# rlawhdrhs/Vision-Transformer-OpenCL

Hardware: AMD Instinct MI355X
Metric: images/sec ViT-B/16 224² fp32 @batch256; % MFMA roofline; top-1 match (higher is better)
Workload: dtype f32; 1 GPU; ViT-B/16 224x224 fp32 forward, batch 256 per GPU, synthetic weights and images (BASELINE.json configs[1]); batch_per_gpu=256, global_batch=256, parallelism=dp1, lanes_per_gpu=1, prune_last_layer=False, ln_fold=True, device=AMD Radeon Graphics, arch=gfx950:sramecc+:xnack-, compute_units=256, clock_mhz=2400

## Files before the change

vision-transformer-opencl_amd/csrc/vit_attention_hd.hip:

```cpp
#include <hip/hip_runtime.h>

#include <math.h>

#include <type_traits>

#include "vit_attention.hpp"
#include "vit_hip_kernels.h"
#include "vit_split3.hpp"

namespace {

using namespace vitattn;
typedef unsigned int u32x2 __attribute__((ext_vector_type(2)));

constexpr int HD_WAVES = 4, HD_THREADS = HD_WAVES * 64;
constexpr int HD_QROWS = HD_WAVES * 32;

template <int HD, bool BF16>
struct Geo {
    typedef typename std::conditional<BF16, bf16_t, float>::type elem;
    static constexpr int VEC = BF16 ? 8 : 4;
    static constexpr int KC = BF16 ? 64 : 32;
    static constexpr int KT = KC / 32;
    static constexpr int DT = (HD + 31) / 32;
    static constexpr int HDK = BF16 ? (HD + 15) / 16 * 16 : HD;
    static constexpr int KROW = HDK + (BF16 ? 8 : 4);
    static constexpr int VROW = KC + 4;
    static constexpr int K_ELEMS = KC * KROW, V_ELEMS = DT * 32 * VROW;
    static constexpr int MIN_WAVES = BF16 && HD <= 96 ? 4 : 3;
};

template <int HD, bool BF16, bool QS>
__global__ __launch_bounds__(HD_THREADS, (Geo<HD, BF16>::MIN_WAVES)) void attention_hd_kernel(
    const typename Geo<HD, BF16>::elem *__restrict__ qkv, typename Geo<HD, BF16>::elem *__restrict__ out, int tokens, int heads, int q_rows,
    int qblocks, float scale) {
    typedef Geo<HD, BF16> G;
    typedef typename G::elem elem;
    constexpr int VEC = G::VEC, KC = G::KC, KT = G::KT, DT = G::DT, KROW = G::KROW, VROW = G::VROW;
    __shared__ __attribute__((aligned(16))) elem Ks[G::K_ELEMS];
    __shared__ __attribute__((aligned(16))) elem Vt[G::V_ELEMS];

    const int tid = threadIdx.x, lane = tid & 63, wave = tid >> 6;
    const int r = lane & 31, h = lane >> 5;
    const int image = blockIdx.x / qblocks, qblock = blockIdx.x - image * qblocks, head = blockIdx.y;
    const size_t D = (size_t)heads * HD, ld = 3 * D;
    const elem *rows = qkv + (size_t)image * tokens * ld + (size_t)head * HD;
    const elem *krows = rows + D, *vrows = rows + 2 * D;
    const int qrow0 = qblock * HD_QROWS + wave * 32;
    const bool active = qrow0 < q_rows;

    constexpr int NQ = BF16 ? G::HDK / 16 : HD / 8;
    typename std::conditional<BF16, bf16x8, f32x4>::type qf[NQ];
    {
        int qrow = qrow0 + r;
        qrow = qrow < q_rows ? qrow : q_rows - 1;
        const elem *qp = rows + (size_t)qrow * ld;
#pragma unroll
        for (int ks = 0; ks < NQ; ++ks) {
            if constexpr (BF16) {
                const int d0 = 16 * ks + 8 * h;
                u32x4 w = {0u, 0u, 0u, 0u};
                if (d0 < HD && active) w = *reinterpret_cast<const u32x4 *>(qp + d0);
                qf[ks] = __builtin_bit_cast(bf16x8, w);
            } else {
                f32x4 w = {0.0f, 0.0f, 0.0f, 0.0f};
                if (active) w = *reinterpret_cast<const f32x4 *>(qp + 8 * ks + 4 * h);
                qf[ks] = w;
            }
        }
    }

    f32x16 o[DT];
#pragma unroll
    for (int dt = 0; dt < DT; ++dt)
#pragma unroll
        for (int v = 0; v < 16; ++v) o[dt][v] = 0.0f;
    float m_run = -INFINITY, l_run = 0.0f;

    for (int key0 = 0; key0 < tokens; key0 += KC) {
        constexpr int KP = G::HDK / VEC;
        for (int i = tid; i < KC * KP; i += HD_THREADS) {
            const int row = i / KP, c = i - row * KP, key = key0 + row;
            u32x4 w = {0u, 0u, 0u, 0u};
            if (key < tokens && c * VEC < HD) w = *reinterpret_cast<const u32x4 *>(krows + (size_t)key * ld + c * VEC);
            *reinterpret_cast<u32x4 *>(Ks + row * KROW + c * VEC) = w;
        }
        constexpr int VP = HD / VEC;
        if constexpr (BF16) {
            for (int i = tid; i < (KC / 2) * VP; i += HD_THREADS) {
                const int c = i / (KC / 2), row = 2 * (i - c * (KC / 2)), key = key0 + row;
                u32x4 a = {0u, 0u, 0u, 0u}, b = {0u, 0u, 0u, 0u};
                if (key < tokens) a = *reinterpret_cast<const u32x4 *>(vrows + (size_t)key * ld + c * VEC);
                if (key + 1 < tokens) b = *reinterpret_cast<const u32x4 *>(vrows + (size_t)(key + 1) * ld + c * VEC);
#pragma unroll
                for (int j = 0; j < 4; ++j) {
                    *reinterpret_cast<unsigned *>(Vt + (c * 8 + 2 * j) * VROW + row) = (a[j] & 0xffffu) | (b[j] << 16);
                    *reinterpret_cast<unsigned *>(Vt + (c * 8 + 2 * j + 1) * VROW + row) = (a[j] >> 16) | (b[j] & 0xffff0000u);
                }
            }
        } else {
            for (int i = tid; i < KC * VP; i += HD_THREADS) {
                const int c = i / KC, row = i - c * KC, key = key0 + row;
                u32x4 w = {0u, 0u, 0u, 0u};
                if (key < tokens) w = *reinterpret_cast<const u32x4 *>(vrows + (size_t)key * ld + c * VEC);
#pragma unroll
                for (int j = 0; j < 4; ++j) Vt[(c * 4 + j) * VROW + row] = __uint_as_float(w[j]);
            }
        }
        __syncthreads();

        if (active) {
#pragma unroll
            for (int t = 0; t < KT; ++t) {
                const int tile0 = key0 + 32 * t;
                if (tile0 >= tokens) break;
                f32x16 s;
#pragma unroll
                for (int v = 0; v < 16; ++v) s[v] = 0.0f;
                const elem *kp = Ks + (32 * t + r) * KROW;
#pragma unroll
                for (int ks = 0; ks < NQ; ++ks) {
                    if constexpr (BF16) {
                        const bf16x8 kf = *reinterpret_cast<const bf16x8 *>(kp + 16 * ks + 8 * h);
                        s = __builtin_amdgcn_mfma_f32_32x32x16_bf16(kf, qf[ks], s, 0, 0, 0);
                    } else {
                        const f32x4 kf = *reinterpret_cast<const f32x4 *>(kp + 8 * ks + 4 * h);
#pragma unroll
                        for (int i = 0; i < 4; ++i) s = __builtin_amdgcn_mfma_f32_32x32x2f32(kf[i], qf[ks][i], s, 0, 0, 0);
                    }
                }
                if (tile0 + 32 > tokens) {
#pragma unroll
                    for (int v = 0; v < 16; ++v) {
                        const int key = tile0 + (v & 3) + 8 * (v >> 2) + 4 * h;
                        s[v] = key < tokens ? s[v] : -INFINITY;
                    }
                }
                float cmax = s[0];
#pragma unroll
                for (int v = 1; v < 16; ++v) cmax = fmaxf(cmax, s[v]);
                cmax = fmaxf(cmax, __shfl_xor(cmax, 32));
                constexpr float kDefer = 8.0f;
                const float m_old = m_run;
                const float m_new = (cmax - m_old) * scale > kDefer ? cmax : m_old;
                const float mneg = -m_new * scale;
                m_run = m_new;
                float sum = 0.0f;
#pragma unroll
                for (int v = 0; v < 16; ++v) {
                    s[v] = __builtin_amdgcn_exp2f(QS ? s[v] + mneg : fmaf(s[v], scale, mneg));
                    sum += s[v];
                }
                if (__any(m_new != m_old)) {
                    const float alpha = __builtin_amdgcn_exp2f((m_old - m_new) * scale);
                    l_run *= alpha;
#pragma unroll
                    for (int dt = 0; dt < DT; ++dt)
#pragma unroll
                        for (int v = 0; v < 16; ++v) o[dt][v] *= alpha;
                }
                l_run += sum;
                if constexpr (BF16) {
#pragma unroll
                    for (int s2 = 0; s2 < 2; ++s2) {
                        bf16x8 pf, pl;
#pragma unroll
                        for (int j = 0; j < 8; ++j) {
                            pf[j] = (__bf16)s[8 * s2 + j];
                            pl[j] = (__bf16)(s[8 * s2 + j] - (float)pf[j]);
                        }
#pragma unroll
                        for (int dt = 0; dt < DT; ++dt) {
                            const bf16_t *vp = Vt + (32 * dt + r) * VROW + 32 * t + 16 * s2 + 4 * h;
                            const u32x2 lo = *reinterpret_cast<const u32x2 *>(vp), hi = *reinterpret_cast<const u32x2 *>(vp + 8);
                            const u32x4 both = {lo[0], lo[1], hi[0], hi[1]};
                            o[dt] = __builtin_amdgcn_mfma_f32_32x32x16_bf16(__builtin_bit_cast(bf16x8, both), pl, o[dt], 0, 0, 0);
                            o[dt] = __builtin_amdgcn_mfma_f32_32x32x16_bf16(__builtin_bit_cast(bf16x8, both), pf, o[dt], 0, 0, 0);
                        }
                    }
                } else {
#pragma unroll
                    for (int q = 0; q < 4; ++q)
#pragma unroll
                        for (int dt = 0; dt < DT; ++dt) {
                            const f32x4 vf = *reinterpret_cast<const f32x4 *>(Vt + (32 * dt + r) * VROW + 32 * t + 8 * q + 4 * h);
#pragma unroll
                            for (int i = 0; i < 4; ++i) o[dt] = __builtin_amdgcn_mfma_f32_32x32x2f32(vf[i], s[4 * q + i], o[dt], 0, 0, 0);
                        }
                }
            }
        }
        __syncthreads();
    }

    const int qrow = qrow0 + r;
    if (active && qrow < q_rows) {
        const float inv = 1.0f / (l_run + __shfl_xor(l_run, 32));
        elem *dst = out + ((size_t)image * tokens + qrow) * D + (size_t)head * HD;
#pragma unroll
        for (int dt = 0; dt < DT; ++dt)
#pragma unroll
            for (int q = 0; q < 4; ++q) {
                const int d0 = 32 * dt + 8 * q + 4 * h;
                if (d0 < HD) {
                    if constexpr (BF16) {
                        bf16x4 w;
#pragma unroll
                        for (int i = 0; i < 4; ++i) w[i] = (__bf16)(o[dt][4 * q + i] * inv);
                        *reinterpret_cast<u32x2 *>(dst + d0) = __builtin_bit_cast(u32x2, w);
                    } else {
                        const f32x4 w = {o[dt][4 * q] * inv, o[dt][4 * q + 1] * inv, o[dt][4 * q + 2] * inv, o[dt][4 * q + 3] * inv};
                        *reinterpret_cast<f32x4 *>(dst + d0) = w;
                    }
                }
            }
    }
}

#ifndef ATT_SPLIT_WAVES
#define ATT_SPLIT_WAVES 4
#endif
#ifndef ATT_SPLIT_MINW
#define ATT_SPLIT_MINW 3
#endif
constexpr int SP_WAVES = ATT_SPLIT_WAVES, SP_THREADS = SP_WAVES * 64, SP_QROWS = SP_WAVES * 32;

__global__ __launch_bounds__(SP_THREADS, ATT_SPLIT_MINW) void attention_split_kernel(const float *__restrict__ qkv, float *__restrict__ out,
                                                                                    int tokens, int heads, int q_rows, int qblocks) {
    using vitsplit::SPLIT_TERM_A;
    using vitsplit::SPLIT_TERM_W;
    using vitsplit::split3_piece8;
    typedef Geo<64, true> G;
    constexpr int HD = 64, KC = G::KC, KT = G::KT, DT = G::DT, KROW = G::KROW, VROW = G::VROW, NQ = HD / 16;
    __shared__ __attribute__((aligned(16))) bf16_t Ks[3 * G::K_ELEMS];
    __shared__ __attribute__((aligned(16))) bf16_t Vt[3 * G::V_ELEMS];

    const int tid = threadIdx.x, lane = tid & 63, wave = tid >> 6;
    const int r = lane & 31, h = lane >> 5;
    const int image = blockIdx.x / qblocks, qblock = blockIdx.x - image * qblocks, head = blockIdx.y;
    const size_t D = (size_t)heads * HD, ld = 3 * D;
    const float *rows = qkv + (size_t)image * tokens * ld + (size_t)head * HD;
    const float *krows = rows + D, *vrows = rows + 2 * D;
    const int qrow0 = qblock * SP_QROWS + wave * 32;
    const bool active = qrow0 < q_rows;
    const f32x4 zero4 = {0.0f, 0.0f, 0.0f, 0.0f};

    bf16x8 qf[3][NQ];
    {
        int qrow = qrow0 + r;
        qrow = qrow < q_rows ? qrow : q_rows - 1;
        const float *qp = rows + (size_t)qrow * ld + 8 * h;
#pragma unroll
        for (int ks = 0; ks < NQ; ++ks) {
            f32x4 x0 = zero4, x1 = zero4;
            if (active) {
                x0 = *reinterpret_cast<const f32x4 *>(qp + 16 * ks);
                x1 = *reinterpret_cast<const f32x4 *>(qp + 16 * ks + 4);
            }
#pragma unroll
            for (int pl = 0; pl < 3; ++pl) qf[pl][ks] = __builtin_bit_cast(bf16x8, split3_piece8(x0, x1, pl));
        }
    }

    f32x16 o[DT];
#pragma unroll
    for (int dt = 0; dt < DT; ++dt)
#pragma unroll
        for (int v = 0; v < 16; ++v) o[dt][v] = 0.0f;
    float m_run = -INFINITY, l_run = 0.0f;

    constexpr int K_ITEMS = KC * (HD / 8), V_ITEMS = (KC / 2) * (HD / 8);
    constexpr int KI = (K_ITEMS + SP_THREADS - 1) / SP_THREADS;
    constexpr int V_TID0 = SP_THREADS > V_ITEMS ? SP_THREADS - V_ITEMS : 0;
    static_assert(V_ITEMS <= SP_THREADS, "one V item per thread at most");
    const int vi = tid - V_TID0;
    f32x4 kx[KI][2], vx[4];
    auto fetch = [&](int key0) {
#pragma unroll
        for (int it = 0; it < KI; ++it) {
            const int i = tid + it * SP_THREADS, row = i / (HD / 8), c = i - row * (HD / 8), key = key0 + row;
            kx[it][0] = kx[it][1] = zero4;
            if (i < K_ITEMS && key < tokens) {
                const float *p = krows + (size_t)key * ld + 8 * c;
                kx[it][0] = *reinterpret_cast<const f32x4 *>(p);
                kx[it][1] = *reinterpret_cast<const f32x4 *>(p + 4);
            }
        }
        if (vi >= 0) {
            const int c = vi / (KC / 2), key = key0 + 2 * (vi - c * (KC / 2));
#pragma unroll
            for (int j = 0; j < 4; ++j) vx[j] = zero4;
            if (key < tokens) {
                const float *p = vrows + (size_t)key * ld + 8 * c;
                vx[0] = *reinterpret_cast<const f32x4 *>(p);
                vx[1] = *reinterpret_cast<const f32x4 *>(p + 4);
            }
            if (key + 1 < tokens) {
                const float *p = vrows + (size_t)(key + 1) * ld + 8 * c;
                vx[2] = *reinterpret_cast<const f32x4 *>(p);
                vx[3] = *reinterpret_cast<const f32x4 *>(p + 4);
            }
        }
    };
    auto store = [&](bf16_t *Kd, bf16_t *Vd) {
#pragma unroll
        for (int it = 0; it < KI; ++it) {
            const int i = tid + it * SP_THREADS, row = i / (HD / 8), c = i - row * (HD / 8);
            if (i < K_ITEMS) {
#pragma unroll
                for (int pl = 0; pl < 3; ++pl)
                    *reinterpret_cast<u32x4 *>(Kd + pl * G::K_ELEMS + row * KROW + 8 * c) = split3_piece8(kx[it][0], kx[it][1], pl);
            }
        }
        if (vi >= 0) {
            const int c = vi / (KC / 2), row = 2 * (vi - c * (KC / 2));
#pragma unroll
            for (int pl = 0; pl < 3; ++pl) {
                const u32x4 a = split3_piece8(vx[0], vx[1], pl), b = split3_piece8(vx[2], vx[3], pl);
                bf16_t *vd = Vd + pl * G::V_ELEMS + (c * 8) * VROW + row;
#pragma unroll
                for (int j = 0; j < 4; ++j) {
                    *reinterpret_cast<unsigned *>(vd + (2 * j) * VROW) = (a[j] & 0xffffu) | (b[j] << 16);
                    *reinterpret_cast<unsigned *>(vd + (2 * j + 1) * VROW) = (a[j] >> 16) | (b[j] & 0xffff0000u);
                }
            }
        }
    };

    for (int key0 = 0; key0 < tokens; key0 += KC) {
        fetch(key0);
        store(Ks, Vt);
        __syncthreads();

        if (active) {
#pragma unroll
            for (int t = 0; t < KT; ++t) {
                const int tile0 = key0 + 32 * t;
                if (tile0 >= tokens) break;
                f32x16 s;
#pragma unroll
                for (int v = 0; v < 16; ++v) s[v] = 0.0f;
                const bf16_t *kp = Ks + (32 * t + r) * KROW + 8 * h;
#pragma unroll
                for (int ks = 0; ks < NQ; ++ks) {
                    bf16x8 kf[3];
#pragma unroll
                    for (int pl = 0; pl < 3; ++pl) kf[pl] = *reinterpret_cast<const bf16x8 *>(kp + pl * G::K_ELEMS + 16 * ks);
#pragma unroll
                    for (int term = 0; term < 6; ++term)
                        s = __builtin_amdgcn_mfma_f32_32x32x16_bf16(kf[SPLIT_TERM_A[term]], qf[SPLIT_TERM_W[term]][ks], s, 0, 0, 0);
                }
                if (tile0 + 32 > tokens) {
#pragma unroll
                    for (int v = 0; v < 16; ++v) {
                        const int key = tile0 + (v & 3) + 8 * (v >> 2) + 4 * h;
                        s[v] = key < tokens ? s[v] : -INFINITY;
                    }
                }
                float cmax = s[0];
#pragma unroll
                for (int v = 1; v < 16; ++v) cmax = fmaxf(cmax, s[v]);
                cmax = fmaxf(cmax, __shfl_xor(cmax, 32));
                constexpr float kDefer = 8.0f, scale = kScale64;
                const float m_old = m_run;
                const float m_new = (cmax - m_old) * scale > kDefer ? cmax : m_old;
                const float mneg = -m_new * scale;
                m_run = m_new;
                float sum = 0.0f;
#pragma unroll
                for (int v = 0; v < 16; ++v) {
                    s[v] = __builtin_amdgcn_exp2f(fmaf(s[v], scale, mneg));
                    sum += s[v];
                }
                if (__any(m_new != m_old)) {
                    const float alpha = __builtin_amdgcn_exp2f((m_old - m_new) * scale);
                    l_run *= alpha;
#pragma unroll
                    for (int dt = 0; dt < DT; ++dt)
#pragma unroll
                        for (int v = 0; v < 16; ++v) o[dt][v] *= alpha;
                }
                l_run += sum;
#pragma unroll
                for (int s2 = 0; s2 < 2; ++s2) {
                    if (tile0 + 16 * s2 >= tokens) break;
                    f32x4 x0 = {s[8 * s2], s[8 * s2 + 1], s[8 * s2 + 2], s[8 * s2 + 3]};
                    f32x4 x1 = {s[8 * s2 + 4], s[8 * s2 + 5], s[8 * s2 + 6], s[8 * s2 + 7]};
                    bf16x8 pf[3], vf[DT][3];
#pragma unroll
                    for (int pl = 0; pl < 3; ++pl) pf[pl] = __builtin_bit_cast(bf16x8, split3_piece8(x0, x1, pl));
#pragma unroll
                    for (int dt = 0; dt < DT; ++dt)
#pragma unroll
                        for (int pl = 0; pl < 3; ++pl) {
                            const bf16_t *vp = Vt + pl * G::V_ELEMS + (32 * dt + r) * VROW + 32 * t + 16 * s2 + 4 * h;
                            const u32x2 lo = *reinterpret_cast<const u32x2 *>(vp), hi = *reinterpret_cast<const u32x2 *>(vp + 8);
                            const u32x4 both = {lo[0], lo[1], hi[0], hi[1]};
                            vf[dt][pl] = __builtin_bit_cast(bf16x8, both);
                        }
#pragma unroll
                    for (int term = 0; term < 6; ++term)
#pragma unroll
                        for (int dt = 0; dt < DT; ++dt)
                            o[dt] = __builtin_amdgcn_mfma_f32_32x32x16_bf16(vf[dt][SPLIT_TERM_A[term]], pf[SPLIT_TERM_W[term]], o[dt], 0, 0, 0);
                }
            }
        }
        __syncthreads();
    }

    const int qrow = qrow0 + r;
    if (active && qrow < q_rows) {
        const float inv = 1.0f / (l_run + __shfl_xor(l_run, 32));
        float *dst = out + ((size_t)image * tokens + qrow) * D + (size_t)head * HD + 4 * h;
#pragma unroll
        for (int dt = 0; dt < DT; ++dt)
#pragma unroll
            for (int q = 0; q < 4; ++q) {
                const f32x4 w = {o[dt][4 * q] * inv, o[dt][4 * q + 1] * inv, o[dt][4 * q + 2] * inv, o[dt][4 * q + 3] * inv};
                *reinterpret_cast<f32x4 *>(dst + 32 * dt + 8 * q) = w;
            }
    }
}

template <bool BF16, bool QS>
int launch_hd(hipStream_t s, const typename Geo<128, BF16>::elem *qkv, typename Geo<128, BF16>::elem *out, int n_images, int tokens,
              int heads, int head_dim, int q_rows) {
    const int qblocks = (q_rows + HD_QROWS - 1) / HD_QROWS;
    if (heads > 65535 || (long long)n_images * qblocks > 0x7fffffffLL) return static_cast<int>(hipErrorInvalidValue);
    const float scale = QS ? 1.0f : vithip_qscale(head_dim);
    return dispatch_int<72, 8, 8>(head_dim, [&](auto hd) {
        hipLaunchKernelGGL((attention_hd_kernel<decltype(hd)::value, BF16, QS>), dim3((unsigned)(n_images * qblocks), (unsigned)heads),
                           dim3(HD_THREADS), 0, s, qkv, out, tokens, heads, q_rows, qblocks, scale);
        return static_cast<int>(hipGetLastError());
    });
}

}

int vitattn::attention_hd_f32(hipStream_t s, const float *qkv, float *out, int n_images, int tokens, int heads, int head_dim, int q_rows) {
    return launch_hd<false, false>(s, qkv, out, n_images, tokens, heads, head_dim, q_rows);
}

int vitattn::attention_hd_bf16(hipStream_t s, const unsigned short *qkv, unsigned short *out, int n_images, int tokens, int heads,
                               int head_dim, int q_rows, bool q_scaled) {
    return q_scaled ? launch_hd<true, true>(s, qkv, out, n_images, tokens, heads, head_dim, q_rows)
                    : launch_hd<true, false>(s, qkv, out, n_images, tokens, heads, head_dim, q_rows);
}

int vitattn::attention_split_f32(hipStream_t s, const float *qkv, float *out, int n_images, int tokens, int heads, int q_rows) {
    const int qblocks = (q_rows + SP_QROWS - 1) / SP_QROWS;
    if (heads > 65535 || (long long)n_images * qblocks > 0x7fffffffLL) return static_cast<int>(hipErrorInvalidValue);
    hipLaunchKernelGGL(attention_split_kernel, dim3((unsigned)(n_images * qblocks), (unsigned)heads), dim3(SP_THREADS), 0, s, qkv, out,
                       tokens, heads, q_rows, qblocks);
    return static_cast<int>(hipGetLastError());
}

extern "C" float vithip_qscale(int head_dim) {
    if (!vitattn::hd_accepted(head_dim)) return 0.0f;
    return (float)((1.0 / sqrt((double)head_dim)) * 1.4426950408889634074);
}
```

Before: 5749 images/sec.

## Store V row-major with swizzle and read via transposing LDS loads; use buffer loads

The split-bf16 attention kernel now stores V in shared memory in its natural key-major layout with an XOR swizzle, and builds MFMA B fragments with a transposing read helper instead of writing V transposed with scattered 32-bit LDS stores. K and V global fetches are unified so every thread loads one K and one V item per pass, using buffer loads with a bounds-limited resource in place of per-item branch checks. The aim is to cut LDS store instructions and bank conflicts and to simplify address arithmetic. It relies on the v_fragment_tr helper and hardware out-of-range zeroing, and drops the compile-time macro overrides.

```diff
diff --git a/vision-transformer-opencl_amd/csrc/vit_attention_hd.hip b/vision-transformer-opencl_amd/csrc/vit_attention_hd.hip
--- a/vision-transformer-opencl_amd/csrc/vit_attention_hd.hip
+++ b/vision-transformer-opencl_amd/csrc/vit_attention_hd.hip
@@ -217,30 +217,25 @@
     }
 }
 
-#ifndef ATT_SPLIT_WAVES
-#define ATT_SPLIT_WAVES 4
-#endif
-#ifndef ATT_SPLIT_MINW
-#define ATT_SPLIT_MINW 3
-#endif
-constexpr int SP_WAVES = ATT_SPLIT_WAVES, SP_THREADS = SP_WAVES * 64, SP_QROWS = SP_WAVES * 32;
-
-__global__ __launch_bounds__(SP_THREADS, ATT_SPLIT_MINW) void attention_split_kernel(const float *__restrict__ qkv, float *__restrict__ out,
-                                                                                    int tokens, int heads, int q_rows, int qblocks) {
+constexpr int SP_WAVES = 4, SP_THREADS = SP_WAVES * 64, SP_QROWS = SP_WAVES * 32;
+constexpr int SP_MINW = 3;
+constexpr int SP_VLD = 64;
+
+__global__ __launch_bounds__(SP_THREADS, SP_MINW) void attention_split_kernel(const float *__restrict__ qkv, float *__restrict__ out, int tokens,
+                                                                             int heads, int q_rows, int qblocks) {
     using vitsplit::SPLIT_TERM_A;
     using vitsplit::SPLIT_TERM_W;
     using vitsplit::split3_piece8;
     typedef Geo<64, true> G;
-    constexpr int HD = 64, KC = G::KC, KT = G::KT, DT = G::DT, KROW = G::KROW, VROW = G::VROW, NQ = HD / 16;
+    constexpr int HD = 64, KC = G::KC, KT = G::KT, DT = G::DT, KROW = G::KROW, NQ = HD / 16, V_ELEMS = KC * SP_VLD;
     __shared__ __attribute__((aligned(16))) bf16_t Ks[3 * G::K_ELEMS];
-    __shared__ __attribute__((aligned(16))) bf16_t Vt[3 * G::V_ELEMS];
+    __shared__ __attribute__((aligned(16))) bf16_t Vs[3 * V_ELEMS];
 
     const int tid = threadIdx.x, lane = tid & 63, wave = tid >> 6;
     const int r = lane & 31, h = lane >> 5;
     const int image = blockIdx.x / qblocks, qblock = blockIdx.x - image * qblocks, head = blockIdx.y;
     const size_t D = (size_t)heads * HD, ld = 3 * D;
     const float *rows = qkv + (size_t)image * tokens * ld + (size_t)head * HD;
-    const float *krows = rows + D, *vrows = rows + 2 * D;
     const int qrow0 = qblock * SP_QROWS + wave * 32;
     const bool active = qrow0 < q_rows;
     const f32x4 zero4 = {0.0f, 0.0f, 0.0f, 0.0f};
@@ -269,67 +264,44 @@
         for (int v = 0; v < 16; ++v) o[dt][v] = 0.0f;
     float m_run = -INFINITY, l_run = 0.0f;
 
-    constexpr int K_ITEMS = KC * (HD / 8), V_ITEMS = (KC / 2) * (HD / 8);
-    constexpr int KI = (K_ITEMS + SP_THREADS - 1) / SP_THREADS;
-    constexpr int V_TID0 = SP_THREADS > V_ITEMS ? SP_THREADS - V_ITEMS : 0;
-    static_assert(V_ITEMS <= SP_THREADS, "one V item per thread at most");
-    const int vi = tid - V_TID0;
-    f32x4 kx[KI][2], vx[4];
+    constexpr int ITEMS = KC * (HD / 8), NI = ITEMS / SP_THREADS;
+    static_assert(ITEMS % SP_THREADS == 0, "every thread has an item of K and one of V in every pass");
+    f32x4 kx[NI][2], vx[NI][2];
+    unsigned xoff[NI];
+#pragma unroll
+    for (int it = 0; it < NI; ++it) {
+        const int j = tid + it * SP_THREADS;
+        xoff[it] = 4u * ((unsigned)(j >> 3) * (unsigned)ld + (unsigned)D + 8u * (j & 7));
+    }
+    const unsigned v_ofs = 4u * (unsigned)D;
     auto fetch = [&](int key0) {
-#pragma unroll
-        for (int it = 0; it < KI; ++it) {
-            const int i = tid + it * SP_THREADS, row = i / (HD / 8), c = i - row * (HD / 8), key = key0 + row;
-            kx[it][0] = kx[it][1] = zero4;
-            if (i < K_ITEMS && key < tokens) {
-                const float *p = krows + (size_t)key * ld + 8 * c;
-                kx[it][0] = *reinterpret_cast<const f32x4 *>(p);
-                kx[it][1] = *reinterpret_cast<const f32x4 *>(p + 4);
-            }
-        }
-        if (vi >= 0) {
-            const int c = vi / (KC / 2), key = key0 + 2 * (vi - c * (KC / 2));
-#pragma unroll
-            for (int j = 0; j < 4; ++j) vx[j] = zero4;
-            if (key < tokens) {
-                const float *p = vrows + (size_t)key * ld + 8 * c;
-                vx[0] = *reinterpret_cast<const f32x4 *>(p);
-                vx[1] = *reinterpret_cast<const f32x4 *>(p + 4);
-            }
-            if (key + 1 < tokens) {
-                const float *p = vrows + (size_t)(key + 1) * ld + 8 * c;
-                vx[2] = *reinterpret_cast<const f32x4 *>(p);
-                vx[3] = *reinterpret_cast<const f32x4 *>(p + 4);
-            }
+        const int valid = tokens - key0 < KC ? tokens - key0 : KC;
+        const unsigned bytes = 4u * ((unsigned)(valid - 1) * (unsigned)ld + 2u * (unsigned)D + HD);
+        const __amdgpu_buffer_rsrc_t rs = __builtin_amdgcn_make_buffer_rsrc(const_cast<float *>(rows + (size_t)key0 * ld), 0, (int)bytes, 0x00020000);
+#pragma unroll
+        for (int it = 0; it < NI; ++it) {
+            kx[it][0] = __builtin_bit_cast(f32x4, __builtin_amdgcn_raw_buffer_load_b128(rs, xoff[it], 0, 0));
+            kx[it][1] = __builtin_bit_cast(f32x4, __builtin_amdgcn_raw_buffer_load_b128(rs, xoff[it], 16, 0));
+            vx[it][0] = __builtin_bit_cast(f32x4, __builtin_amdgcn_raw_buffer_load_b128(rs, xoff[it], v_ofs, 0));
+            vx[it][1] = __builtin_bit_cast(f32x4, __builtin_amdgcn_raw_buffer_load_b128(rs, xoff[it], v_ofs + 16, 0));
         }
     };
-    auto store = [&](bf16_t *Kd, bf16_t *Vd) {
-#pragma unroll
-        for (int it = 0; it < KI; ++it) {
-            const int i = tid + it * SP_THREADS, row = i / (HD / 8), c = i - row * (HD / 8);
-            if (i < K_ITEMS) {
-#pragma unroll
-                for (int pl = 0; pl < 3; ++pl)
-                    *reinterpret_cast<u32x4 *>(Kd + pl * G::K_ELEMS + row * KROW + 8 * c) = split3_piece8(kx[it][0], kx[it][1], pl);
-            }
-        }
-        if (vi >= 0) {
-            const int c = vi / (KC / 2), row = 2 * (vi - c * (KC / 2));
+    auto store = [&]() {
+#pragma unroll
+        for (int it = 0; it < NI; ++it) {
+            const int j = tid + it * SP_THREADS, row = j >> 3, c = j & 7;
+            bf16_t *kd = Ks + row * KROW + 8 * c, *vd = Vs + row * SP_VLD + 8 * (c ^ (4 * ((row >> 1) & 1)));
 #pragma unroll
             for (int pl = 0; pl < 3; ++pl) {
-                const u32x4 a = split3_piece8(vx[0], vx[1], pl), b = split3_piece8(vx[2], vx[3], pl);
-                bf16_t *vd = Vd + pl * G::V_ELEMS + (c * 8) * VROW + row;
-#pragma unroll
-                for (int j = 0; j < 4; ++j) {
-                    *reinterpret_cast<unsigned *>(vd + (2 * j) * VROW) = (a[j] & 0xffffu) | (b[j] << 16);
-                    *reinterpret_cast<unsigned *>(vd + (2 * j + 1) * VROW) = (a[j] >> 16) | (b[j] & 0xffff0000u);
-                }
+                *reinterpret_cast<u32x4 *>(kd + pl * G::K_ELEMS) = split3_piece8(kx[it][0], kx[it][1], pl);
+                *reinterpret_cast<u32x4 *>(vd + pl * V_ELEMS) = split3_piece8(vx[it][0], vx[it][1], pl);
             }
         }
     };
 
     for (int key0 = 0; key0 < tokens; key0 += KC) {
         fetch(key0);
-        store(Ks, Vt);
+        store();
         __syncthreads();
 
         if (active) {
@@ -386,18 +358,14 @@
                     if (tile0 + 16 * s2 >= tokens) break;
                     f32x4 x0 = {s[8 * s2], s[8 * s2 + 1], s[8 * s2 + 2], s[8 * s2 + 3]};
                     f32x4 x1 = {s[8 * s2 + 4], s[8 * s2 + 5], s[8 * s2 + 6], s[8 * s2 + 7]};
-                    bf16x8 pf[3], vf[DT][3];
+                    bf16x8 pf[3];
 #pragma unroll
                     for (int pl = 0; pl < 3; ++pl) pf[pl] = __builtin_bit_cast(bf16x8, split3_piece8(x0, x1, pl));
+                    bf16x8 vf[DT][3];
 #pragma unroll
                     for (int dt = 0; dt < DT; ++dt)
 #pragma unroll
-                        for (int pl = 0; pl < 3; ++pl) {
-                            const bf16_t *vp = Vt + pl * G::V_ELEMS + (32 * dt + r) * VROW + 32 * t + 16 * s2 + 4 * h;
-                            const u32x2 lo = *reinterpret_cast<const u32x2 *>(vp), hi = *reinterpret_cast<const u32x2 *>(vp + 8);
-                            const u32x4 both = {lo[0], lo[1], hi[0], hi[1]};
-                            vf[dt][pl] = __builtin_bit_cast(bf16x8, both);
-                        }
+                        for (int pl = 0; pl < 3; ++pl) vf[dt][pl] = v_fragment_tr<SP_VLD>(Vs + pl * V_ELEMS, 32 * t + 16 * s2, dt, lane);
 #pragma unroll
                     for (int term = 0; term < 6; ++term)
 #pragma unroll
```

After: 5776 images/sec (median of 3 runs). No clear change (+0.5%).
